# EnterpriseCV-6/Season-NeRF

Measured on AMD Instinct MI355X. Metric: ray-samples/sec (4096 rays x 96 samples forward render, T_NeRF 8x256), higher is better.
Workload: dtype i8x3 (16-bit fixed point as two int8 digits on v_mfma_i32_32x32x32_i8, exact int32 accumulate, fp32 epilogue)

## Files before the change

season_nerf_amd/csrc/kernels_i8x2.hip:

```cpp
#include <type_traits>

#include "mlp_i8_device.h"

namespace snerf {

constexpr int NW2 = 8;
constexpr int TILE2 = 32 * NW2;
constexpr int DMA_WAVES2 = 4, PIECES4 = kChunkBytes / kFragBytes / DMA_WAVES2;
constexpr int RING2_D = 7;
constexpr int PFX = 2;
static_assert(PIECES4 == 4 && kChunkPairs == 8, "dma_chunk4 moves four pieces per loading wave; barrier positions assume 8-pair chunks");

struct Ring2 {
    uint32_t wr;
    uint32_t goff;
    uint32_t cur;
};
__device__ __forceinline__ uint32_t ring2_next(uint32_t off) {
    off += kChunkBytes;
    return off == RING2_D * kChunkBytes ? 0u : off;
}
__device__ __forceinline__ void dma_chunk4(const uint8_t* stream, uint32_t goff, lds_char* lds, uint32_t wr, int wave, int lane) {
    const uint8_t* b0 = stream + goff + wave * (4 * kFragBytes);
    const uint32_t dst = (uint32_t)(uintptr_t)(lds + wr + wave * (4 * kFragBytes));
    const uint32_t voff = lane * 16;
    uint32_t keep;
    asm volatile(
        "s_mov_b32 %0, m0\n\t"
        "s_mov_b32 m0, %2\n\t"
        "s_nop 0\n\t"
        "global_load_lds_dwordx4 %1, %3\n\t"
        "s_add_u32 m0, m0, 0x400\n\t"
        "s_nop 0\n\t"
        "global_load_lds_dwordx4 %1, %4\n\t"
        "s_add_u32 m0, m0, 0x400\n\t"
        "s_nop 0\n\t"
        "global_load_lds_dwordx4 %1, %5\n\t"
        "s_add_u32 m0, m0, 0x400\n\t"
        "s_nop 0\n\t"
        "global_load_lds_dwordx4 %1, %6\n\t"
        "s_mov_b32 m0, %0"
        : "=&s"(keep)
        : "v"(voff), "s"(dst), "s"(b0), "s"(b0 + kFragBytes), "s"(b0 + 2 * kFragBytes), "s"(b0 + 3 * kFragBytes)
        : "memory", "scc");
}

template <int PHASE>
__device__ __forceinline__ void ring_step2(Ring2& rg, const uint8_t* stream, uint32_t stream_bytes, lds_char* lds, int wave, int lane) {
#if defined(SNERF_ABLATE) && (ABL & 4)
    return;
#endif
    if (PHASE == 0) {
        asm volatile("s_waitcnt vmcnt(%0)\n\ts_barrier" ::"n"((RING2_D - 3) * PIECES4) : "memory");
        dma_chunk4(stream, rg.goff, lds, rg.wr, wave, lane);
    } else {
        asm volatile("s_barrier" ::: "memory");
    }
    rg.goff += kChunkBytes;
    if (rg.goff >= stream_bytes) rg.goff = 0;
    rg.wr = ring2_next(rg.wr);
}

struct TabQ {
    f32x4 sc, bi;
};
__device__ __forceinline__ TabQ load_tab_quad(lds_cfloat* tab_l, int b, int h, int g) {
    typedef volatile const __attribute__((address_space(3))) f32x4 lds_vf32x4;
    lds_vf32x4* tp = (lds_vf32x4*)(tab_l + (b * 2 + h) * 32);
    TabQ t;
    t.sc = tp[g];
    t.bi = tp[4 + g];
    return t;
}
__device__ __forceinline__ TabQ load_tab_quad_h(lds_cfloat* tab_h, int b, int g) {
    typedef volatile const __attribute__((address_space(3))) f32x4 lds_vf32x4;
    lds_vf32x4* tp = (lds_vf32x4*)(tab_h + b * 64);
    TabQ t;
    t.sc = tp[g];
    t.bi = tp[4 + g];
    return t;
}
template <int TAB_, int NB_, bool SIN_, bool RAWL_, bool DEP_>
struct Carry {
    static constexpr bool on = true, SIN = SIN_, RAWL = RAWL_, DEP = DEP_;
    static constexpr int TAB = TAB_, NB = NB_;
};
struct NoCarry {
    static constexpr bool on = false, SIN = false, RAWL = false, DEP = false;
    static constexpr int TAB = 0, NB = 1;
};
__host__ __device__ constexpr bool carry_fits(int nb, bool dep) { return !dep || nb >= 2; }
struct CarryDst {
    Frag8* out;
    f32x16* raw;
    const float* rawx;
};

struct Boundary {
    int m[16];
    i32x4 fT[PFX], fL[PFX];
};

template <bool SIN, bool RAWL>
__device__ __forceinline__ void epi_quad(const int* m, int g, const TabQ& t, const f32x4* rqg, const float* rawx, Frag8* ob, f32x16* raw) {
    float v[4];
#if defined(SNERF_ABLATE) && (ABL & 16)
#pragma unroll
    for (int j = 0; j < 4; ++j) v[j] = __builtin_bit_cast(float, (m[4 * g + j] & 0x007fffff) | 0x3f000000) - 0.75f;
#else
#pragma unroll
    for (int j = 0; j < 4; ++j) v[j] = __builtin_fmaf((float)m[4 * g + j], t.sc[j], t.bi[j]);
    if constexpr (RAWL) {
#pragma unroll
        for (int j = 0; j < 4; ++j)
            v[j] = __builtin_fmaf(rqg[0][j], rawx[0], __builtin_fmaf(rqg[1][j], rawx[1], __builtin_fmaf(rqg[2][j], rawx[2], v[j])));
    }
#endif
    if constexpr (SIN) {
#if defined(SNERF_ABLATE) && (ABL & 8)
#pragma unroll
        for (int j = 0; j < 4; ++j) v[j] = __builtin_fmaf(__builtin_amdgcn_fractf(v[j]), 2.f, -1.f);
#elif !(defined(SNERF_ABLATE) && (ABL & 16))
#pragma unroll
        for (int j = 0; j < 4; ++j) v[j] = sin2pi(v[j]);
#endif
        int hi, lo;
        digits4(v[0], v[1], v[2], v[3], hi, lo);
        asm volatile("" : "+v"(hi), "+v"(lo));
        ob->hi[g] = hi;
        ob->lo[g] = lo;
    } else {
#pragma unroll
        for (int j = 0; j < 4; ++j) (*raw)[4 * g + j] = v[j];
    }
}

__host__ __device__ constexpr bool field_feeds_next(int l) { return l != F_HEAD && l != F_S4; }
static_assert(F_S1 == F_HEAD + 1 && F_A1 == F_S4 + 1 && F_FC1 == 0, "the kernels' LAYER macros build the carry of layer L from layer L - 1");
__host__ __device__ constexpr int field_last(int variant) { return variant == 0 ? F_AC : variant == 1 ? F_S4 : F_HEAD; }
__host__ __device__ constexpr bool field_carries(int W, int variant, int C, int l) {
    return l != field_last(variant) && carry_fits(prog_layer(PROG_FIELD, W, C, l, FMT_I8).n_out / 32, field_feeds_next(l));
}

#if defined(SNERF_ABLATE) && (ABL & 2)
constexpr bool kNoFragReads = true;
#else
constexpr bool kNoFragReads = false;
#endif
#define REQUEST(QN, SLOT)                                                                              \
    do {                                                                                               \
        if ((QN) % kChunkPairs == 0) {                                                                 \
            ring_step2<PHASE>(rg, stream, stream_bytes, lds, wave, lane);                              \
            if ((QN) > 0) rg.cur = ring2_next(rg.cur);                                                 \
        }                                                                                              \
        lds_char* ap_ = lds + rg.cur + ((QN) % kChunkPairs) * kPairBytes + lane * 16;                  \
        if (!kNoFragReads) {                                                                           \
            fT[SLOT] = *(lds_ci32x4*)ap_;                                                              \
            fL[SLOT] = *(lds_ci32x4*)(ap_ + kFragBytes);                                               \
        } else {                                                                                       \
            asm volatile("" : "+v"(fT[SLOT]), "+v"(fL[SLOT]));                                         \
        }                                                                                              \
    } while (0)
#define REQUEST_NEXT(J, SLOT)                                                                          \
    do {                                                                                               \
        if ((J) == 0) {                                                                                \
            ring_step2<PHASE>(rg, stream, stream_bytes, lds, wave, lane);                              \
            rg.cur = ring2_next(rg.cur);                                                               \
        }                                                                                              \
        lds_char* ap_ = lds + rg.cur + (J) * kPairBytes + lane * 16;                                   \
        if (!kNoFragReads) {                                                                           \
            fT[SLOT] = *(lds_ci32x4*)ap_;                                                              \
            fL[SLOT] = *(lds_ci32x4*)(ap_ + kFragBytes);                                               \
        } else {                                                                                       \
            asm volatile("" : "+v"(fT[SLOT]), "+v"(fL[SLOT]));                                         \
        }                                                                                              \
    } while (0)

template <int NB, int KS0, int KS1, bool SIN, bool RAWL = false, int PHASE = 0, bool OPQ = false, class PEND = NoCarry, bool HANDOFF = false, bool PRE_IN = false,
          bool PRE_OUT = false>
__device__ __forceinline__ void run_layer8x2(Ring2& rg, const uint8_t* stream, uint32_t stream_bytes, lds_char* lds, lds_cfloat* tab0, lds_cfloat* tab_l,
                                             const Frag8* in0, const Frag8* in1, Frag8* out, f32x16* raw, Boundary& bd, const CarryDst& pd,
                                             int wave, int lane, const float* rawx = nullptr) {
    constexpr int KS = KS0 + KS1, NP = NB * KS;
    constexpr int NBP = PEND::NB;
    static_assert(!PRE_OUT || (NP >= PFX && NP % PFX == 0), "the successor expects its pair j in fragment slot j");
    static_assert(!PRE_IN || NP >= PFX, "the predecessor requested PFX pairs of this layer");
    int (&m)[16] = bd.m;
    i32x4 (&fT)[PFX] = bd.fT;
    i32x4 (&fL)[PFX] = bd.fL;
    static_assert(!PEND::on || carry_fits(NBP, PEND::DEP), "a carried block that is the operand of k-step 0 has no k-step to run in");
    static_assert(!(PEND::on && PEND::DEP) || NBP <= KS0, "Carry::DEP: the producer's output is in0");
    typedef volatile const __attribute__((address_space(3))) f32x4 lds_vf32x4;
    f32x4 rq[4][3];
    const int h = lane >> 5;
    lds_cfloat* ptab_l = tab0 + PEND::TAB;
    lds_cfloat* base_h = (PEND::on ? ptab_l : tab_l) + 32 * h;
    if constexpr (OPQ) asm volatile("" : "+v"(base_h));
    lds_cfloat* raw_l = tab_l + 2 * 32 * NB;
    lds_cfloat* raw_h = raw_l + 48 * h;
    lds_cfloat* praw_l = ptab_l + 2 * 32 * NBP;
    lds_cfloat* praw_h = praw_l + 48 * h;
    if constexpr (OPQ) asm volatile("" : "+v"(raw_h));
    if constexpr (OPQ && PEND::RAWL) asm volatile("" : "+v"(praw_h));
    lds_cfloat* tab_h = base_h + (tab_l - (PEND::on ? ptab_l : tab_l));
    lds_cfloat* ptab_h = base_h;
    auto tabq = [&](int b_, int g_) { return OPQ ? load_tab_quad_h(tab_h, b_, g_) : load_tab_quad(tab_l, b_, h, g_); };
    auto ptabq = [&](int g_) { return OPQ ? load_tab_quad_h(ptab_h, NBP - 1, g_) : load_tab_quad(ptab_l, NBP - 1, h, g_); };
    if constexpr (kNoFragReads) {
#pragma unroll
        for (int q = 0; q < PFX; ++q) { fT[q] = i32x4{lane, 1, 2, 3}; fL[q] = i32x4{4, lane, 6, 7}; }
    }
    if constexpr (!PRE_IN) {
#pragma unroll
        for (int q = 0; q < PFX; ++q) {
            if (q < NP) REQUEST(q, q);
        }
    }
    Acc8 acc;
    TabQ tq[4];
    auto load_rq = [&](int g, int b_of) {
        if constexpr (RAWL) {
            lds_vf32x4* tp = OPQ ? (lds_vf32x4*)(raw_h + (b_of * 8 + g) * 12) : (lds_vf32x4*)(raw_l + ((b_of * 2 + h) * 4 + g) * 12);
            rq[g][0] = tp[0]; rq[g][1] = tp[1]; rq[g][2] = tp[2];
        }
    };
    auto load_prq = [&](int g) {
        if constexpr (PEND::RAWL) {
            lds_vf32x4* tp = OPQ ? (lds_vf32x4*)(praw_h + ((NBP - 1) * 8 + g) * 12) : (lds_vf32x4*)(praw_l + (((NBP - 1) * 2 + h) * 4 + g) * 12);
            rq[g][0] = tp[0]; rq[g][1] = tp[1]; rq[g][2] = tp[2];
        }
    };
    auto quad = [&](int g, int b_of, const TabQ& t) { epi_quad<SIN, RAWL>(m, g, t, rq[g], rawx, out + b_of, raw); };
    auto pquad = [&](int g, const TabQ& t) { epi_quad<PEND::SIN, PEND::RAWL>(m, g, t, rq[g], pd.rawx, pd.out + (NBP - 1), pd.raw); };
    auto slot = [](int g, bool carried) constexpr { return carried && PEND::DEP ? (g * (NBP - 1)) / 4 : (g * KS) / 4; };
#pragma unroll
    for (int b = 0; b < NB; ++b) {
        const bool carried = b == 0;
        if (b > 0 || PEND::on) {
            if (b > 0) {
                tq[0] = tabq(b - 1, 0);
                load_rq(0, b - 1);
#pragma unroll
                for (int i = 0; i < 16; ++i) m[i] = (int)(((uint32_t)acc.M[i] << 8) + (uint32_t)acc.X[i]);
            } else {
                tq[0] = ptabq(0);
                load_prq(0);
            }
            asm volatile("" ::: "memory");
            __builtin_amdgcn_sched_barrier(0);
        }
#pragma unroll
        for (int i = 0; i < 16; ++i) { acc.M[i] = 0; acc.X[i] = 0; }
#pragma unroll
        for (int s = 0; s < KS; ++s) {
            const int q = b * KS + s;
            const i32x4 aT = fT[q % PFX], aL = fL[q % PFX];
            if (((s + PHASE) & 1) == 0) __builtin_amdgcn_s_setprio(0); else __builtin_amdgcn_s_setprio(3);
            if (q + PFX < NP) REQUEST(q + PFX, q % PFX);
            else if constexpr (PRE_OUT) REQUEST_NEXT(q + PFX - NP, q % PFX);
            if (b > 0 || PEND::on) {
#pragma unroll
                for (int g = 1; g < 4; ++g) {
                    const int sg = slot(g, carried), lg = sg > 0 ? sg - 1 : 0;
                    if (lg == s) {
                        if (b > 0) { tq[g] = tabq(b - 1, g); load_rq(g, b - 1); }
                        else { tq[g] = ptabq(g); load_prq(g); }
                    }
                }
            }
            mfma_i8x3(aT, aL, s < KS0 ? in0[s] : in1[s - KS0], acc);
            if (b > 0 || PEND::on) {
#pragma unroll
                for (int g = 0; g < 4; ++g)
                    if (slot(g, carried) == s) {
                        if (b > 0) quad(g, b - 1, tq[g]);
                        else pquad(g, tq[g]);
                    }
            }
            asm volatile("" ::: "memory");
            __builtin_amdgcn_sched_barrier(0);
        }
    }
#pragma unroll
    for (int i = 0; i < 16; ++i) m[i] = (int)(((uint32_t)acc.M[i] << 8) + (uint32_t)acc.X[i]);
    if constexpr (HANDOFF) {
        asm volatile("" ::: "memory");
        __builtin_amdgcn_sched_barrier(0);
    } else {
#pragma unroll
        for (int g = 0; g < 4; ++g) {
            asm volatile("" ::: "memory");
            const TabQ t = tabq(NB - 1, g);
            load_rq(g, NB - 1);
            quad(g, NB - 1, t);
            asm volatile("" ::: "memory");
            __builtin_amdgcn_sched_barrier(0);
        }
    }
    if constexpr (!PRE_OUT) rg.cur = ring2_next(rg.cur);
}

struct BoundaryK {
    int m[8];
    i32x4 fT[PFX], fL[PFX];
};
struct CarryDstK {
    FragK* out;
    float* raw;
    const float (*rawx)[3];
};
__host__ __device__ constexpr bool carry_fits_k64(int nb, bool dep) { return !dep || nb >= 5; }
__host__ __device__ constexpr bool field_carries_k64(int W, int variant, int C, int l) {
    return l != field_last(variant) && carry_fits_k64(k64_blocks(k64_layer(W, C, l)), field_feeds_next(l));
}
template <bool SIN, bool RAWL>
__device__ __forceinline__ void epi_quad_k64(const int* m, int cg, const TabQ& t, const f32x4* rq, const float (*rawx)[3], FragK* ob, int dw, float* raw) {
    float v[4];
#pragma unroll
    for (int j = 0; j < 4; ++j) v[j] = __builtin_fmaf((float)m[4 * cg + j], t.sc[j], t.bi[j]);
    if constexpr (RAWL) {
#pragma unroll
        for (int j = 0; j < 4; ++j)
            v[j] = __builtin_fmaf(rq[0][j], rawx[cg][0], __builtin_fmaf(rq[1][j], rawx[cg][1], __builtin_fmaf(rq[2][j], rawx[cg][2], v[j])));
    }
    if constexpr (SIN) {
#pragma unroll
        for (int j = 0; j < 4; ++j) v[j] = sin2pi(v[j]);
        int hi, lo;
        digits4(v[0], v[1], v[2], v[3], hi, lo);
        asm volatile("" : "+v"(hi), "+v"(lo));
        ob->hi[cg][dw] = hi;
        ob->lo[cg][dw] = lo;
    } else {
#pragma unroll
        for (int j = 0; j < 4; ++j) raw[4 * cg + j] = v[j];
    }
}

template <int NB, int KS0, int KS1, bool SIN, bool RAWL = false, int PHASE = 0, class PEND = NoCarry, bool HANDOFF = false, bool PRE_IN = false,
          bool PRE_OUT = false>
__device__ __forceinline__ void run_layer16(Ring2& rg, const uint8_t* stream, uint32_t stream_bytes, lds_char* lds, lds_cfloat* tab0, lds_cfloat* tab_l,
                                            const FragK* in0, const FragK* in1, FragK* out, float* raw, BoundaryK& bd, const CarryDstK& pd,
                                            int wave, int lane, const float (*rawx)[3] = nullptr) {
    constexpr int KS = KS0 + KS1, NP = NB * KS;
    constexpr int NBP = PEND::NB;
    static_assert(!PRE_OUT || (NP >= PFX && NP % PFX == 0), "the successor expects its pair j in fragment slot j");
    static_assert(!PRE_IN || NP >= PFX, "the predecessor requested PFX pairs of this layer");
    static_assert(!PEND::on || carry_fits_k64(NBP, PEND::DEP), "a carried block that is an operand of k-step 0 has no k-step to run in");
    static_assert(!(PEND::on && PEND::DEP) || NBP == 4 * KS0, "Carry::DEP: the producer's output is in0");
    int (&m)[8] = bd.m;
    i32x4 (&fT)[PFX] = bd.fT;
    i32x4 (&fL)[PFX] = bd.fL;
    typedef volatile const __attribute__((address_space(3))) f32x4 lds_vf32x4;
    int g = lane >> 4;
    asm volatile("" : "+v"(g));
    lds_cfloat* ptab_l = tab0 + PEND::TAB;
    lds_cfloat* lo_l = PEND::on ? ptab_l : tab_l;
    lds_cfloat* base_g = lo_l + 8 * g;
    lds_cfloat* rbase_g = lo_l + 12 * g;
    const int d_own = (int)(tab_l - lo_l);
    auto tabq = [&](int b_) {
        lds_vf32x4* tp = (lds_vf32x4*)(base_g + d_own + b_ * 32);
        TabQ t;
        t.sc = tp[0];
        t.bi = tp[1];
        return t;
    };
    auto ptabq = [&]() {
        lds_vf32x4* tp = (lds_vf32x4*)(base_g + (NBP - 1) * 32);
        TabQ t;
        t.sc = tp[0];
        t.bi = tp[1];
        return t;
    };
    f32x4 rq[3];
    auto load_rq = [&](int b_of) {
        if constexpr (RAWL) {
            lds_vf32x4* tp = (lds_vf32x4*)(rbase_g + d_own + 2 * 16 * NB + b_of * 48);
            rq[0] = tp[0]; rq[1] = tp[1]; rq[2] = tp[2];
        }
    };
    auto load_prq = [&]() {
        if constexpr (PEND::RAWL) {
            lds_vf32x4* tp = (lds_vf32x4*)(rbase_g + 2 * 16 * NBP + (NBP - 1) * 48);
            rq[0] = tp[0]; rq[1] = tp[1]; rq[2] = tp[2];
        }
    };
    if constexpr (kNoFragReads) {
#pragma unroll
        for (int q = 0; q < PFX; ++q) { fT[q] = i32x4{lane, 1, 2, 3}; fL[q] = i32x4{4, lane, 6, 7}; }
    }
    if constexpr (!PRE_IN) {
#pragma unroll
        for (int q = 0; q < PFX; ++q) {
            if (q < NP) REQUEST(q, q);
        }
    }
    AccK acc;
    TabQ tq;
    auto quad = [&](int cg, int b_of) { epi_quad_k64<SIN, RAWL>(m, cg, tq, rq, rawx, out + b_of / 4, b_of % 4, raw); };
    auto pquad = [&](int cg) { epi_quad_k64<PEND::SIN, PEND::RAWL>(m, cg, tq, rq, pd.rawx, pd.out + (NBP - 1) / 4, (NBP - 1) % 4, pd.raw); };
    auto slot = [](int cg, bool carried) constexpr { return carried && PEND::DEP ? (cg * ((NBP - 1) / 4) * 2) / 3 : (cg * KS) / 2; };
#pragma unroll
    for (int b = 0; b < NB; ++b) {
        const bool carried = b == 0;
        if (b > 0 || PEND::on) {
            if (b > 0) {
                tq = tabq(b - 1);
                load_rq(b - 1);
#pragma unroll
                for (int i = 0; i < 8; ++i) m[i] = (int)(((uint32_t)acc.M[i >> 2][i & 3] << 8) + (uint32_t)acc.X[i >> 2][i & 3]);
            } else {
                tq = ptabq();
                load_prq();
            }
            asm volatile("" ::: "memory");
            __builtin_amdgcn_sched_barrier(0);
        }
#pragma unroll
        for (int cg = 0; cg < 2; ++cg)
#pragma unroll
            for (int i = 0; i < 4; ++i) { acc.M[cg][i] = 0; acc.X[cg][i] = 0; }
#pragma unroll
        for (int s = 0; s < KS; ++s) {
            const int q = b * KS + s;
            const i32x4 aT = fT[q % PFX], aL = fL[q % PFX];
            if (((s + PHASE) & 1) == 0) __builtin_amdgcn_s_setprio(0); else __builtin_amdgcn_s_setprio(3);
            if (q + PFX < NP) REQUEST(q + PFX, q % PFX);
            else if constexpr (PRE_OUT) REQUEST_NEXT(q + PFX - NP, q % PFX);
            mfma_k64x3(aT, aL, s < KS0 ? in0[s] : in1[s - KS0], acc);
            if (b > 0 || PEND::on) {
#pragma unroll
                for (int cg = 0; cg < 2; ++cg)
                    if (slot(cg, carried) == s) {
                        if (b > 0) quad(cg, b - 1);
                        else pquad(cg);
                    }
            }
            asm volatile("" ::: "memory");
            __builtin_amdgcn_sched_barrier(0);
        }
    }
#pragma unroll
    for (int i = 0; i < 8; ++i) m[i] = (int)(((uint32_t)acc.M[i >> 2][i & 3] << 8) + (uint32_t)acc.X[i >> 2][i & 3]);
    if constexpr (HANDOFF) {
        asm volatile("" ::: "memory");
        __builtin_amdgcn_sched_barrier(0);
    } else {
        asm volatile("" ::: "memory");
        tq = tabq(NB - 1);
        load_rq(NB - 1);
#pragma unroll
        for (int cg = 0; cg < 2; ++cg) {
            quad(cg, NB - 1);
            asm volatile("" ::: "memory");
            __builtin_amdgcn_sched_barrier(0);
        }
    }
    if constexpr (!PRE_OUT) rg.cur = ring2_next(rg.cur);
}
#undef REQUEST
#undef REQUEST_NEXT

__host__ __device__ constexpr bool k64_built(int W) { return W == 256; }
bool i8x2_k64_built(int W, int variant) { return variant >= 0 && variant <= 3 && k64_built(W); }

template <int W, int VARIANT, int PHASE>
__device__ __forceinline__ void field_tiles2(const MlpArgs& A, Ring2& rg, lds_char* lds, __attribute__((address_space(3))) float* tab_lds,
                                             int wave, int lane);
template <int W, int VARIANT, int PHASE>
__device__ __forceinline__ void field_tiles16(const MlpArgs& A, Ring2& rg, lds_char* lds, __attribute__((address_space(3))) float* tab_lds,
                                              int wave, int lane);

template <int W, int VARIANT>
__global__ __launch_bounds__(64 * NW2, 1) void mlp_i8x2_kernel(const MlpArgs A) {
    extern __shared__ __attribute__((aligned(16))) char smem[];
    constexpr int C_MAX = kMaxClasses;
    constexpr int W2 = W / 2;
    lds_char* lds = (lds_char*)smem;
    __attribute__((address_space(3))) float* tab_lds = (__attribute__((address_space(3))) float*)(lds + RING2_D * kChunkBytes);

    const int lane = threadIdx.x & 63;
    const int wave = __builtin_amdgcn_readfirstlane(threadIdx.x >> 6);
    const int h = lane >> 5;
    const int C = A.n_classes;

    for (int i = threadIdx.x; i < A.bias_floats; i += 64 * NW2) tab_lds[i] = A.bias[i];

    Ring2 rg;
    rg.cur = 0;
    rg.goff = 0;
    {
        uint32_t wr = 0;
#pragma unroll
        for (int c = 0; c < RING2_D - 2; ++c) {
            if (wave < DMA_WAVES2) dma_chunk4(A.stream, rg.goff, lds, wr, wave, lane);
            rg.goff += kChunkBytes;
            if (rg.goff >= A.stream_bytes) rg.goff = 0;
            wr += kChunkBytes;
        }
        rg.wr = wr;
    }
    __syncthreads();

    bool k64 = false;
    if constexpr (k64_built(W)) k64 = A.k64 != 0;
    if (k64) {
        if constexpr (k64_built(W)) {
            if (wave < 4) field_tiles16<W, VARIANT, 0>(A, rg, lds, tab_lds, wave, lane);
            else field_tiles16<W, VARIANT, 1>(A, rg, lds, tab_lds, wave, lane);
        }
    } else {
        if (wave < 4) field_tiles2<W, VARIANT, 0>(A, rg, lds, tab_lds, wave, lane);
        else field_tiles2<W, VARIANT, 1>(A, rg, lds, tab_lds, wave, lane);
    }
    asm volatile("s_waitcnt vmcnt(0)" ::: "memory");
}

template <int W, int VARIANT, int PHASE>
__device__ __forceinline__ void field_tiles16(const MlpArgs& A, Ring2& rg, lds_char* lds, __attribute__((address_space(3))) float* tab_lds,
                                              int wave, int lane) {
    constexpr int C_MAX = kMaxClasses;
    constexpr int W2 = W / 2;
    const int h = lane >> 5, gq = lane >> 4;
    const int C = A.n_classes;
    const int64_t n_tiles = field_tiles(A.n, VARIANT, TILE2, NW2);
    const int passes = VARIANT == 3 ? (A.n_samples + 31) / 32 : 1;
    int pass = 0;
    RaySum rs;
    for (int64_t tile = blockIdx.x; tile < n_tiles;) {
        const int64_t n = tile * TILE2 + wave * 32 + (lane & 31);
        const bool valid = n < A.n;
        const int64_t nc = valid ? n : A.n - 1;
        const int64_t g = VARIANT == 3 ? 0 : nc / A.group_size;

        float x0, x1, x2;
        if constexpr (VARIANT == 3) raysum_point(rs, A, tile, NW2, wave, pass, lane, x0, x1, x2);
        else field_point(A, nc, x0, x1, x2);
        float s0, s1, s2, pcls[C_MAX];
        field_tile_inputs<VARIANT>(A, g, s0, s1, s2, pcls);
        float rx_p[2][3], rx_s[2][3];
        k64_two_points(x0, x1, x2, lane, rx_p);
        FragK pe;
        make_pe_pos_k64(rx_p, gq, pe);

        constexpr int KW = W / 64, KW2 = W2 / 64;
        FragK hA[KW], hB[KW];
        float raw[8];
        BoundaryK bd;
#define SHAPE(L) k64_layer(W, C_MAX, L)
#define TAB(L) k64_table_start(W, C_MAX, L)
#define HAND(L) (L >= F_FC1 && field_carries_k64(W, VARIANT, C_MAX, L))
#define PEND_T(P) std::conditional_t<HAND(P), Carry<TAB(P), k64_blocks(SHAPE(P)), layer_sine(SHAPE(P)), layer_reads_raw(SHAPE(P)), field_feeds_next(P)>, NoCarry>
#define LAYER(L, IN0, IN1, OUT, RAW, RX, PO, PR, PX)                                                                                                 \
    run_layer16<k64_blocks(SHAPE(L)), SHAPE(L).ks0, SHAPE(L).ks1, layer_sine(SHAPE(L)), layer_reads_raw(SHAPE(L)), PHASE, PEND_T(L - 1), HAND(L),   \
                L != F_FC1, L != field_last(VARIANT)>(rg, A.stream, A.stream_bytes, lds, tab_lds, tab_lds + TAB(L), IN0, IN1, OUT, RAW, bd,         \
                                                      (CarryDstK{PO, PR, PX}), wave, lane, RX)
        FragK x1f[KW2];
        I8_TRUNK(LAYER, &pe, hA, hB, x1f, raw, rx_p,
                 if constexpr (VARIANT != 3) {
                     const bool up = (lane & 16) != 0;
                     x0 = up ? rx_p[1][0] : rx_p[0][0]; x1 = up ? rx_p[1][1] : rx_p[0][1]; x2 = up ? rx_p[1][2] : rx_p[0][2];
                 });
        float col_r, col_g, col_b, rho_raw;
        float sv_raw = 0.f;
        float adj[3 * C_MAX];
#pragma unroll
        for (int i = 0; i < 3 * C_MAX; ++i) adj[i] = 0.f;
#define HEAD_OUT() col_r = k64_head_row(raw, 0, lane), col_g = k64_head_row(raw, 1, lane), col_b = k64_head_row(raw, 2, lane), rho_raw = k64_head_row(raw, 3, lane)
        if constexpr (VARIANT <= 1) {
            k64_two_points(s0, s1, s2, lane, rx_s);
            FragK ps;
            make_pe_sun_k64(rx_s, gq, ps);
            FragK sA[KW2], sB[KW2];
            I8_SOLAR(LAYER, x1f, &ps, sA, sB, raw, rx_s, HEAD_OUT(););
            if constexpr (VARIANT == 1) sv_raw = k64_head_row(raw, 0, lane);
        } else {
            HEAD_OUT();
        }
        if constexpr (VARIANT == 0) {
            I8_ADJUST(LAYER, x1f, hA, hB, raw, sv_raw = k64_head_row(raw, 0, lane););
#pragma unroll
            for (int i = 0; i < 3 * C_MAX; ++i) adj[i] = k64_head_row(raw, i, lane);
        }
#undef HEAD_OUT
#undef LAYER
#undef PEND_T
#undef HAND
#undef TAB
#undef SHAPE
        if constexpr (VARIANT == 3) {
            RAYSUM_PASS_END(rs, A, tile, pass, passes, NW2, wave, wave, NW2, true, lane, rho_raw, x0, x1, x2, tab_lds + A.bias_floats);
        } else {
            if (h == 0 && valid) store_field_outputs<VARIANT>(A.out, n, C, x0, x1, x2, col_r, col_g, col_b, rho_raw, sv_raw, adj, pcls);
            tile += gridDim.x;
        }
    }
    __builtin_amdgcn_s_setprio(0);
}

template <int W, int VARIANT, int PHASE>
__device__ __forceinline__ void field_tiles2(const MlpArgs& A, Ring2& rg, lds_char* lds, __attribute__((address_space(3))) float* tab_lds,
                                             int wave, int lane) {
    constexpr int C_MAX = kMaxClasses;
    constexpr int W2 = W / 2;
    const int h = lane >> 5;
    const int C = A.n_classes;
    const int64_t n_tiles = field_tiles(A.n, VARIANT, TILE2, NW2);
    const int passes = VARIANT == 3 ? (A.n_samples + 31) / 32 : 1;
    int pass = 0;
    RaySum rs;
    for (int64_t tile = blockIdx.x; tile < n_tiles;) {
        const int64_t n = tile * TILE2 + wave * 32 + (lane & 31);
        const bool valid = n < A.n;
        const int64_t nc = valid ? n : A.n - 1;
        const int64_t g = VARIANT == 3 ? 0 : nc / A.group_size;

        float x0, x1, x2;
        if constexpr (VARIANT == 3) raysum_point(rs, A, tile, NW2, wave, pass, lane, x0, x1, x2);
        else field_point(A, nc, x0, x1, x2);
        float s0, s1, s2, pcls[C_MAX];
        field_tile_inputs<VARIANT>(A, g, s0, s1, s2, pcls);
        Frag8 pe[PEPOS_KS8];
        make_pe_pos8<VARIANT == 3>(x0, x1, x2, h, pe);

        constexpr int KW = W / 32, KW2 = W2 / 32;
        Frag8 hA[KW], hB[KW];
        f32x16 raw;
        Boundary bd;
#define SHAPE(L) field_layer(W, C_MAX, L, FMT_I8)
#define TAB(L) prog_table_start(PROG_FIELD, W, C_MAX, L)
#define HAND(L) (L >= F_FC1 && field_carries(W, VARIANT, C_MAX, L))
#define PEND_T(P) std::conditional_t<HAND(P), Carry<TAB(P), SHAPE(P).nb(), layer_sine(SHAPE(P)), layer_reads_raw(SHAPE(P)), field_feeds_next(P)>, NoCarry>
        constexpr bool XPF = KW2 >= PFX && KW2 % PFX == 0;
#define LAYER(L, IN0, IN1, OUT, RAW, RX, PO, PR, PX)                                                                                                 \
    run_layer8x2<SHAPE(L).nb(), SHAPE(L).ks0, SHAPE(L).ks1, layer_sine(SHAPE(L)), layer_reads_raw(SHAPE(L)), PHASE, VARIANT == 3, PEND_T(L - 1), HAND(L), \
                 XPF && L != F_FC1, XPF && L != field_last(VARIANT)>(rg, A.stream, A.stream_bytes, lds, tab_lds, tab_lds + TAB(L), IN0, IN1, OUT, RAW, bd, \
                                                                     (CarryDst{PO, PR, PX}), wave, lane, RX)
        const float rx_p[3] = {x0, x1, x2}, rx_s[3] = {s0, s1, s2};
        Frag8 x1f[KW2];
        I8_TRUNK(LAYER, pe, hA, hB, x1f, &raw, rx_p);
        float col_r, col_g, col_b, rho_raw;
        float sv_raw = 0.f;
        float adj[3 * C_MAX];
#pragma unroll
        for (int i = 0; i < 3 * C_MAX; ++i) adj[i] = 0.f;
        if constexpr (VARIANT <= 1) {
            Frag8 ps[PESUN_KS8];
            make_pe_sun8(s0, s1, s2, h, ps);
            Frag8 sA[KW2], sB[KW2];
            I8_SOLAR(LAYER, x1f, ps, sA, sB, &raw, rx_s, col_r = raw[0], col_g = raw[1], col_b = raw[2], rho_raw = raw[3];);
            if constexpr (VARIANT == 1) sv_raw = raw[0];
        } else {
            col_r = raw[0], col_g = raw[1], col_b = raw[2], rho_raw = raw[3];
        }
        if constexpr (VARIANT == 0) {
            I8_ADJUST(LAYER, x1f, hA, hB, &raw, sv_raw = raw[0];);
#pragma unroll
            for (int i = 0; i < 3 * C_MAX; ++i) adj[i] = raw[i];
        }
#undef LAYER
#undef PEND_T
#undef HAND
#undef TAB
#undef SHAPE
        if constexpr (VARIANT == 3) {
            RAYSUM_PASS_END(rs, A, tile, pass, passes, NW2, wave, wave, NW2, true, lane, rho_raw, x0, x1, x2, tab_lds + A.bias_floats);
        } else {
            if (h == 0 && valid) store_field_outputs<VARIANT>(A.out, n, C, x0, x1, x2, col_r, col_g, col_b, rho_raw, sv_raw, adj, pcls);
            tile += gridDim.x;
        }
    }
    __builtin_amdgcn_s_setprio(0);
}

template <int W, int VARIANT>
static hipError_t launch_mlp_i8x2_t(const MlpArgs& a, int n_cu, hipStream_t st) {
    return launch_fused(mlp_i8x2_kernel<W, VARIANT>, field_tiles(a.n, VARIANT, TILE2, NW2), 64 * NW2,
                        RING2_D * kChunkBytes + a.bias_floats * 4 + kVoteBytes, a, n_cu, st);
}

hipError_t launch_mlp_i8x2(int W, int variant, const MlpArgs& a, int n_cu, hipStream_t st) {
#define CASE(Wv)                                                              \
    if (W == Wv) {                                                            \
        if (variant == 0) return launch_mlp_i8x2_t<Wv, 0>(a, n_cu, st);       \
        if (variant == 1) return launch_mlp_i8x2_t<Wv, 1>(a, n_cu, st);       \
        if (variant == 3) return launch_mlp_i8x2_t<Wv, 3>(a, n_cu, st);       \
        return launch_mlp_i8x2_t<Wv, 2>(a, n_cu, st);                         \
    }
    CASE(64)
    CASE(256)
#undef CASE
    return hipErrorInvalidValue;
}

}
```

Baseline: 549.0 million.

## Load bias table by direct LDS DMA and defer ring prefill past first tile inputs

The bias/scale table is now copied into LDS with global_load_lds by the four DMA waves, replacing the per-thread load/store loop. The prologue now issues only the first weight chunk and drops the block-wide __syncthreads. The remaining prefill chunks are issued by the loading waves after the first tile's point and input values are in registers, so those global reads are not queued behind the prefill. This shortens the per-block startup latency. It relies on later vmcnt waits and barriers to order the table and ring data, and it adds a launch-time check that the table size is a multiple of 4 floats and at least one fragment.

New measurement: 545.6 million. No clear change (-0.6%).

```diff
diff --git a/season_nerf_amd/csrc/kernels_i8x2.hip b/season_nerf_amd/csrc/kernels_i8x2.hip
--- a/season_nerf_amd/csrc/kernels_i8x2.hip
+++ b/season_nerf_amd/csrc/kernels_i8x2.hip
@@ -45,6 +45,27 @@
         : "memory", "scc");
 }
 
+__device__ __forceinline__ void dma_piece(const uint8_t* src, uint32_t dst, int lane) {
+    const uint32_t voff = lane * 16;
+    uint32_t keep;
+    asm volatile(
+        "s_mov_b32 %0, m0\n\t"
+        "s_mov_b32 m0, %2\n\t"
+        "s_nop 0\n\t"
+        "global_load_lds_dwordx4 %1, %3\n\t"
+        "s_mov_b32 m0, %0"
+        : "=&s"(keep)
+        : "v"(voff), "s"(dst), "s"(src)
+        : "memory");
+}
+__device__ __forceinline__ void dma_table(const float* table, int table_floats, lds_char* tab_lds, int wave, int lane) {
+    const uint32_t bytes = (uint32_t)table_floats * 4, last = bytes - kFragBytes;
+    for (uint32_t off = wave * kFragBytes; off < bytes; off += DMA_WAVES2 * kFragBytes) {
+        const uint32_t o = off < last ? off : last;
+        dma_piece((const uint8_t*)table + o, (uint32_t)(uintptr_t)(tab_lds + o), lane);
+    }
+}
+
 template <int PHASE>
 __device__ __forceinline__ void ring_step2(Ring2& rg, const uint8_t* stream, uint32_t stream_bytes, lds_char* lds, int wave, int lane) {
 #if defined(SNERF_ABLATE) && (ABL & 4)
@@ -59,6 +80,26 @@
     rg.goff += kChunkBytes;
     if (rg.goff >= stream_bytes) rg.goff = 0;
     rg.wr = ring2_next(rg.wr);
+}
+
+template <int PHASE>
+__device__ __forceinline__ void ring_start_rest(bool& start, const MlpArgs& A, lds_char* lds, int wave, int lane, float x0, float x1, float x2, float s0,
+                                                float s1, float s2, const float* pcls) {
+    static_assert(kMaxClasses == 5, "the asm below names every class probability");
+    if constexpr (PHASE == 0) {
+        if (start) {
+            asm volatile("" ::"v"(x0), "v"(x1), "v"(x2), "v"(s0), "v"(s1), "v"(s2), "v"(pcls[0]), "v"(pcls[1]), "v"(pcls[2]), "v"(pcls[3]), "v"(pcls[4])
+                         : "memory");
+            uint32_t goff = 0;
+#pragma unroll
+            for (int c = 1; c < RING2_D - 2; ++c) {
+                goff += kChunkBytes;
+                if (goff >= A.stream_bytes) goff = 0;
+                dma_chunk4(A.stream, goff, lds, c * kChunkBytes, wave, lane);
+            }
+        }
+    }
+    start = false;
 }
 
 struct TabQ {
@@ -485,23 +526,19 @@
     const int h = lane >> 5;
     const int C = A.n_classes;
 
-    for (int i = threadIdx.x; i < A.bias_floats; i += 64 * NW2) tab_lds[i] = A.bias[i];
-
+    if (wave < DMA_WAVES2) {
+        dma_table(A.bias, A.bias_floats, (lds_char*)tab_lds, wave, lane);
+        dma_chunk4(A.stream, 0, lds, 0, wave, lane);
+    }
     Ring2 rg;
     rg.cur = 0;
     rg.goff = 0;
-    {
-        uint32_t wr = 0;
-#pragma unroll
-        for (int c = 0; c < RING2_D - 2; ++c) {
-            if (wave < DMA_WAVES2) dma_chunk4(A.stream, rg.goff, lds, wr, wave, lane);
-            rg.goff += kChunkBytes;
-            if (rg.goff >= A.stream_bytes) rg.goff = 0;
-            wr += kChunkBytes;
-        }
-        rg.wr = wr;
-    }
-    __syncthreads();
+    rg.wr = (RING2_D - 2) * kChunkBytes;
+#pragma unroll
+    for (int c = 0; c < RING2_D - 2; ++c) {
+        rg.goff += kChunkBytes;
+        if (rg.goff >= A.stream_bytes) rg.goff = 0;
+    }
 
     bool k64 = false;
     if constexpr (k64_built(W)) k64 = A.k64 != 0;
@@ -528,6 +565,7 @@
     const int passes = VARIANT == 3 ? (A.n_samples + 31) / 32 : 1;
     int pass = 0;
     RaySum rs;
+    bool start = true;
     for (int64_t tile = blockIdx.x; tile < n_tiles;) {
         const int64_t n = tile * TILE2 + wave * 32 + (lane & 31);
         const bool valid = n < A.n;
@@ -543,6 +581,7 @@
         k64_two_points(x0, x1, x2, lane, rx_p);
         FragK pe;
         make_pe_pos_k64(rx_p, gq, pe);
+        ring_start_rest<PHASE>(start, A, lds, wave, lane, x0, x1, x2, s0, s1, s2, pcls);
 
         constexpr int KW = W / 64, KW2 = W2 / 64;
         FragK hA[KW], hB[KW];
@@ -610,6 +649,7 @@
     const int passes = VARIANT == 3 ? (A.n_samples + 31) / 32 : 1;
     int pass = 0;
     RaySum rs;
+    bool start = true;
     for (int64_t tile = blockIdx.x; tile < n_tiles;) {
         const int64_t n = tile * TILE2 + wave * 32 + (lane & 31);
         const bool valid = n < A.n;
@@ -623,6 +663,7 @@
         field_tile_inputs<VARIANT>(A, g, s0, s1, s2, pcls);
         Frag8 pe[PEPOS_KS8];
         make_pe_pos8<VARIANT == 3>(x0, x1, x2, h, pe);
+        ring_start_rest<PHASE>(start, A, lds, wave, lane, x0, x1, x2, s0, s1, s2, pcls);
 
         constexpr int KW = W / 32, KW2 = W2 / 32;
         Frag8 hA[KW], hB[KW];
@@ -676,6 +717,7 @@
 
 template <int W, int VARIANT>
 static hipError_t launch_mlp_i8x2_t(const MlpArgs& a, int n_cu, hipStream_t st) {
+    if (a.bias_floats % 4 != 0 || a.bias_floats * 4 < kFragBytes) return hipErrorInvalidValue;
     return launch_fused(mlp_i8x2_kernel<W, VARIANT>, field_tiles(a.n, VARIANT, TILE2, NW2), 64 * NW2,
                         RING2_D * kChunkBytes + a.bias_floats * 4 + kVoteBytes, a, n_cu, st);
 }
```
